# vismaychuriwala/Fast-Image-Editing-with-Generative-Models

Measured on AMD Instinct MI355X. Metric: PIE-Bench images/sec @1024^2 SSD-1B fp16 4-step, higher is better.
Workload: dtype f16; 1 GPU; ssd-1b fp16 + ControlNet-Canny(full) LCM img2img, num_inference_steps=4, strength=0.5, guidance=1.5, 1024x1024, batch=1 image per GPU, one edit at a time; unet_preset=ssd-1b-A1, controlnet_preset=controlnet-canny-sdxl-full, unet_evals=2, cfg_batch=2, parallelism=image-parallel x1, launch=hipGraph replay, weights=f16

## Files before the change

### fast-image-editing-with-generative-models_amd/csrc/gemm_common.h

```cpp
#pragma once
#include "fie_internal.h"
#include "gemm_addr.h"

namespace fie_gemm {

constexpr int BK = 64;

struct GemmArgs {
    const half_t* A1; int64_t lda1; int K1;
    const half_t* A2; int64_t lda2;
    const half_t* A3; int64_t lda3; int C2x, C3x; int64_t a3_bytes;
    int H, W, Cin, OH, OW, stride, pt, pl, ups;
    const half_t* Wt; int64_t ldw;
    half_t* C; int64_t ldc;
    int M, N, K;
    const half_t* bias;
    const half_t* rowbias; int64_t ld_rowbias; int rows_per_batch;
    const half_t* res; int64_t ldr;
    float scale; int act;
    int nbm, nbn;
    int64_t a1_bytes, a2_bytes, w_bytes;
    int taps2, oscat, opy, opx;
    int64_t w_par_stride;
    int gn_nch, gn_chunk0;
// ... 398 lines not shown
                    const float vq = lane == 0 ? tq[0] : lane == 1 ? tq[1] : lane == 2 ? tq[2] : tq[3];
                    float2* dst = reinterpret_cast<float2*>(p.gn_partial) + ((int64_t)b * nch + chunk) * p.gn_G + nfrag / p.gn_cg + lane;
                    *dst = make_float2(vs, vq);
                }
            }
        }
    }
    if constexpr (BUF) {
        if (p.out_f8) {
            const __amdgpu_buffer_rsrc_t rs8 = buf_rsrc(p.C, (int64_t)(p.M - 1) * p.ldc + (geglu ? p.N >> 1 : p.N));
            const float inv = p.out_inv_scale;
            auto q = [&](float x) { return fie_sat448(x * inv); };
#pragma unroll
            for (int j = 0; j < FM; ++j) {
                const int m = mrow + j * fld;
                const unsigned ro = m < p.M ? (unsigned)m * (unsigned)p.ldc : kRowOut;
#pragma unroll
                for (int i = 0; i < FN; ++i) {
                    const int n = ncol + i * 16;
                    if (geglu) {
                        const int pk = __builtin_amdgcn_cvt_pk_fp8_f32(q(acc[i][j][0]), q(acc[i][j][1]), 0, false);
                        __builtin_amdgcn_raw_buffer_store_b16((unsigned short)(pk & 0xffff), rs8, ro + (n < p.N ? (unsigned)(n >> 1) : kColOut), 0, 0);
                    } else {
                        int pk = __builtin_amdgcn_cvt_pk_fp8_f32(q(acc[i][j][0]), q(acc[i][j][1]), 0, false);
                        pk = __builtin_amdgcn_cvt_pk_fp8_f32(q(acc[i][j][2]), q(acc[i][j][3]), pk, true);
                        __builtin_amdgcn_raw_buffer_store_b32((unsigned)pk, rs8, ro + (n < p.N ? (unsigned)n : kColOut), 0, 0);
                    }
                }
            }
            return;
        }
    }
    const __amdgpu_buffer_rsrc_t rs_c = buf_rsrc(p.C, BUF ? ((int64_t)(p.oscat ? 4 * (int64_t)p.M : p.M) - 1) * p.ldc * 2 + (geglu ? p.N >> 1 : p.N) * 2 : 0);
#pragma unroll
    for (int j = 0; j < FM; ++j) {
        const int m = mrow + j * fld;
        const unsigned ro = coff_row(j);
#pragma unroll
        for (int i = 0; i < FN; ++i) {
            const int n = ncol + i * 16;
            if (geglu) {
                f16x2 o;
                o[0] = (half_t)acc[i][j][0]; o[1] = (half_t)acc[i][j][1];
                if constexpr (BUF) {
                    unsigned bits; __builtin_memcpy(&bits, &o, 4);
                    __builtin_amdgcn_raw_buffer_store_b32(bits, rs_c, ro + coff(i, true), 0, 0);
                } else if (m < p.M && n < p.N) {
                    *reinterpret_cast<f16x2*>(p.C + (int64_t)m * p.ldc + (n >> 1)) = o;
                }
            } else {
                f16x4 o;
#pragma unroll
                for (int r = 0; r < 4; ++r) o[r] = (half_t)acc[i][j][r];
                if constexpr (BUF) {
                    u32x2 bits; __builtin_memcpy(&bits, &o, 8);
                    __builtin_amdgcn_raw_buffer_store_b64(bits, rs_c, ro + coff(i, false), 0, 0);
                } else if (m < p.M && n < p.N) {
                    *reinterpret_cast<f16x4*>(p.C + (int64_t)m * p.ldc + n) = o;
                }
            }
        }
        __builtin_amdgcn_sched_barrier(0);
    }
}

constexpr unsigned kOob = 0x80000000u;

__device__ __forceinline__ void bload16(__amdgpu_buffer_rsrc_t rsrc, half_t* lds_dst, unsigned voff, unsigned soff) {
    __builtin_amdgcn_raw_ptr_buffer_load_lds(rsrc, (__attribute__((address_space(3))) void*)lds_dst, 16, voff, soff, 0, 0);
}

template <int N>
__device__ __forceinline__ void wait_vm() {
    static_assert(N >= 0 && N < 64, "vmcnt is a 6-bit counter");
    asm volatile("s_waitcnt vmcnt(%0)" ::"n"(N) : "memory");
}

template <int N>
__device__ __forceinline__ void wait_vm_barrier() {
    static_assert(N >= 0 && N < 64, "vmcnt is a 6-bit counter");
    asm volatile("s_waitcnt vmcnt(%0)\n\ts_barrier" ::"n"(N) : "memory");
}

template <int FM, int FN, int NW>
__device__ __forceinline__ bool splitk_reduce(const GemmArgs& p, f32x4 (&acc)[FN][FM], int tile, int slice, int tid, void* lds) {
    constexpr int kTile = FM * FN * NW * 64 * 4;
    const int S = p.splitk;
    float* base = p.sk_slabs + (size_t)tile * S * kTile;
    {
        const __amdgpu_buffer_rsrc_t rs = buf_rsrc(base + (size_t)slice * kTile, kTile * 4);
#pragma unroll
        for (int i = 0; i < FN; ++i)
#pragma unroll
            for (int j = 0; j < FM; ++j)
                __builtin_amdgcn_raw_buffer_store_b128(__builtin_bit_cast(u32x4, acc[i][j]), rs, (unsigned)((i * FM + j) * NW * 64 + tid) * 16u, 0, 16);
    }
    asm volatile("s_waitcnt vmcnt(0)" ::: "memory");
    __syncthreads();
    volatile unsigned* flag = reinterpret_cast<volatile unsigned*>(lds);
    if (tid == 0) *flag = __hip_atomic_fetch_add(p.sk_tickets + tile, 1u, __ATOMIC_RELAXED, __HIP_MEMORY_SCOPE_AGENT);
    __syncthreads();
    if (*flag % (unsigned)S != (unsigned)(S - 1)) return false;
    if (tid == 0) {
        (void)__hip_atomic_fetch_sub(p.sk_tickets + tile, (unsigned)S, __ATOMIC_RELAXED, __HIP_MEMORY_SCOPE_AGENT);
        __builtin_amdgcn_fence(__ATOMIC_ACQUIRE, "agent");
    }
    asm volatile("s_waitcnt vmcnt(0)" ::: "memory");
    __syncthreads();
#pragma unroll
    for (int i = 0; i < FN; ++i)
#pragma unroll
        for (int j = 0; j < FM; ++j) acc[i][j] = (f32x4){0.f, 0.f, 0.f, 0.f};
    for (int s = 0; s < S; ++s) {
        const __amdgpu_buffer_rsrc_t rs = buf_rsrc(base + (size_t)s * kTile, kTile * 4);
        u32x4 v[FN][FM];
#pragma unroll
        for (int i = 0; i < FN; ++i)
#pragma unroll
            for (int j = 0; j < FM; ++j) v[i][j] = __builtin_amdgcn_raw_buffer_load_b128(rs, (unsigned)((i * FM + j) * NW * 64 + tid) * 16u, 0, 16);
#pragma unroll
        for (int i = 0; i < FN; ++i)
#pragma unroll
            for (int j = 0; j < FM; ++j) acc[i][j] += __builtin_bit_cast(f32x4, v[i][j]);
    }
    return true;
}

__device__ __forceinline__ int xcd_remap(int bid, int nwg) {
    const int q = nwg >> 3, r = nwg & 7, xcd = bid & 7;
    return (xcd < r ? xcd * (q + 1) : r * (q + 1) + (xcd - r) * q) + (bid >> 3);
}

}

int fie_launch_gemm8(fie_ctx* ctx, const fie_gemm::GemmArgs& a, int conv, int split);
int fie_gemm8_init(void);
int fie_gemm_init(void);
int fie_launch_conv_halo(fie_ctx* ctx, fie_gemm::GemmArgs& a, int stamped);
bool fie_conv_halo_ok(const fie_gemm::GemmArgs& a);
bool fie_conv_halo_edge_ok(const fie_gemm::GemmArgs& a);
int64_t fie_conv_halo_patches(const fie_gemm::GemmArgs& a);
int fie_launch_conv_thin(fie_ctx* ctx, fie_gemm::GemmArgs& a);
bool fie_conv_thin_ok(const fie_gemm::GemmArgs& a);
bool fie_conv_halo_gna_ok(const fie_gemm::GemmArgs& a);
int fie_conv_halo_init(void);
int fie_launch_gemm_w8(fie_ctx* ctx, const fie_gemm::GemmArgs& a, int conv, int code);
int fie_gemm_w8_init(void);
int fie_launch_gemm_x8(fie_ctx* ctx, const fie_gemm::GemmArgs& a, int code, int conv);
int fie_gemm_x8_init(void);
```

### fast-image-editing-with-generative-models_amd/csrc/gemm_conv.hip

```cpp
#include <algorithm>
#include <cstdio>
#include <cstdlib>
#include <cstring>
#include <utility>

#include "gemm_common.h"
#include "gemm_tiles.h"

using namespace fie_gemm;

namespace {

template <int BM, int BN, int MODE>
__global__ __launch_bounds__(256) void gemm_kernel(GemmArgs p) {
    constexpr int WM = BM / 2, WN = BN / 2;
    constexpr int FM = WM / 16, FN = WN / 16;
    constexpr int RA = BM / 32, RW = BN / 32;
    __shared__ __attribute__((aligned(16))) half_t smem[2 * (BM + BN) * BK];

    const int tid = threadIdx.x;
    const int lane = tid & 63, wave = tid >> 6;
    const int wm = wave & 1, wn = wave >> 1;

    const int bid = xcd_remap(blockIdx.x, gridDim.x);
// ... 38 lines not shown
            }
            ci += BK;
            while (ci >= p.Cin) { ci -= p.Cin; ++tap; }
        } else {
            const bool k1 = k < p.K1;
            const half_t* src = k1 ? p.A1 : p.A2;
            const int64_t ld = k1 ? p.lda1 : p.lda2;
            const int kk = k1 ? k : k - p.K1;
#pragma unroll
            for (int i = 0; i < RA; ++i) {
                const bool ok = a_row[i].ok && k < p.K;
                ra[i] = ok ? *reinterpret_cast<const f16x8*>(src + a_base[i] * ld + kk) : zero8;
            }
        }
#pragma unroll
        for (int i = 0; i < RW; ++i)
            rw[i] = *reinterpret_cast<const f16x8*>(p.Wt + (int64_t)(n0 + r0 + 32 * i) * p.ldw + k);
    };
    auto store_tiles = [&](int buf) {
        half_t* sa = smem + buf * (BM + BN) * BK;
        half_t* sw = sa + BM * BK;
#pragma unroll
        for (int i = 0; i < RA; ++i) *reinterpret_cast<f16x8*>(sa + lds_off(r0 + 32 * i, c8)) = ra[i];
#pragma unroll
        for (int i = 0; i < RW; ++i) *reinterpret_cast<f16x8*>(sw + lds_off(r0 + 32 * i, c8)) = rw[i];
    };

    f32x4 acc[FN][FM];
#pragma unroll
    for (int i = 0; i < FN; ++i)
#pragma unroll
        for (int j = 0; j < FM; ++j) acc[i][j] = (f32x4){0.f, 0.f, 0.f, 0.f};

    const int nk = (p.K + BK - 1) / BK;
    load_tiles(0);
    store_tiles(0);
    __syncthreads();

    const int fr = lane & 15, fq = lane >> 4;
    for (int kt = 0; kt < nk; ++kt) {
        const int buf = kt & 1;
        if (kt + 1 < nk) load_tiles(kt + 1);
        const half_t* sa = smem + buf * (BM + BN) * BK;
        const half_t* sw = sa + BM * BK;
#pragma unroll
        for (int kk = 0; kk < 2; ++kk) {
            f16x8 fw[FN], fa[FM];
#pragma unroll
            for (int i = 0; i < FN; ++i)
                fw[i] = *reinterpret_cast<const f16x8*>(sw + lds_off(wn * WN + i * 16 + fr, kk * 4 + fq));
#pragma unroll
            for (int j = 0; j < FM; ++j)
                fa[j] = *reinterpret_cast<const f16x8*>(sa + lds_off(wm * WM + j * 16 + fr, kk * 4 + fq));
#pragma unroll
            for (int i = 0; i < FN; ++i)
#pragma unroll
                for (int j = 0; j < FM; ++j)
                    acc[i][j] = __builtin_amdgcn_mfma_f32_16x16x32_f16(fw[i], fa[j], acc[i][j], 0, 0, 0);
        }
        if (kt + 1 < nk) store_tiles(buf ^ 1);
        __syncthreads();
    }

    epilogue<FM, FN, WM, WN>(p, acc, m0, n0, wm, wn, lane);
}

template <int NP, int ST>
__device__ __forceinline__ void wait_stage(int later) {
    if (ST >= 3 && later >= 1) wait_vm_barrier<(ST >= 3 ? 1 : 0) * NP>();
    else wait_vm_barrier<0>();
}

template <int OFF>
__device__ __forceinline__ f16x8 lds_read16_async(unsigned addr) {
    f16x8 v;
    asm volatile("ds_read_b128 %0, %1 offset:%2" : "=v"(v) : "v"(addr), "n"(OFF));
    return v;
}
template <int N, int... I>
__device__ __forceinline__ void read_frags(f16x8 (&f)[N], unsigned addr, std::integer_sequence<int, I...>) {
    ((f[I] = lds_read16_async<I * 16 * BK * 2>(addr)), ...);
}

template <int BM, int BN, int ST, int MODE, int NW, bool PF = false, bool STAMP = false, bool ALT = false, int LEAN = 0>
__global__ __launch_bounds__(NW * 64) void gemm3_kernel(GemmArgs p) {
    constexpr bool LNF = LEAN == 2;
    static_assert(!LNF || (MODE == 0 && !STAMP), "LayerNorm fold: GEMM view only");
    static_assert(!ALT || (NW == 8 && MODE == 0 && !PF && !STAMP), "ALT: 8-wave GEMM-view tiles without the fragment prefetch");
    constexpr int WGN = (LEAN == 2 && BM * BN / (NW * 256) <= 16 && (BM / NW) % 16 == 0) ? 1 : (BN / (NW / 2)) % 16 == 0 ? NW / 2 : 1, WGM = NW / WGN;
    constexpr int WM = BM / WGM, WN = BN / WGN;
    constexpr int FM = WM / 16, FN = WN / 16;
    constexpr int NPW = BN / 8;
    constexpr int RA = BM / (8 * NW), RW = (NPW + NW - 1) / NW;
    constexpr int NP = RA + RW;
    constexpr int STAGE = (BM + BN) * BK;
    extern __shared__ __attribute__((aligned(16))) half_t smem[];

    const int tid = threadIdx.x;
    const int lane = tid & 63;
    const int wave = __builtin_amdgcn_readfirstlane(tid >> 6);
    const int wm = wave % WGM, wn = wave / WGM;

    const int bid_all = xcd_remap(blockIdx.x, gridDim.x);
    const int nsplit = p.splitk > 1 ? p.splitk : 1;
    const int tile_all = bid_all / nsplit, slice = bid_all - tile_all * nsplit;
    const int bid = take_parity(p, tile_all);
    const int m0 = (p.order ? bid % p.nbm : bid / p.nbn) * BM;
    const int n0 = (p.order ? bid / p.nbm : bid % p.nbn) * BN;
    const int lr = lane >> 3;
    const int c8 = (lane & 7) ^ lr;

    const int live = p.probe == 1 ? 0 : 1;
    const __amdgpu_buffer_rsrc_t rs_a1 = buf_rsrc(p.A1, (int)p.a1_bytes * live);
    const __amdgpu_buffer_rsrc_t rs_a2 = buf_rsrc(p.A2, (int)p.a2_bytes * live);
    const __amdgpu_buffer_rsrc_t rs_w = buf_rsrc(p.Wt, (int)p.w_bytes * live);
    const __amdgpu_buffer_rsrc_t rs_a3 = buf_rsrc(p.A3, (int)p.a3_bytes * live);
    const int lm0 = p.probe == 2 ? 0 : m0, ln0 = p.probe == 2 ? 0 : n0;

    unsigned a_off1[RA], a_off2[RA];
    unsigned a_off3[RA];
    const ConvGeom g = conv_geom(p, p.taps2);
    ConvRow a_row[RA];
    unsigned a_img[RA];
#pragma unroll
    for (int i = 0; i < RA; ++i) {
        const int m = lm0 + (wave + NW * i) * 8 + lr;
        if (MODE == 2) {
            a_row[i] = conv_row(g, m);
            a_img[i] = (unsigned)a_row[i].b * (unsigned)(p.H * p.W) * (unsigned)p.Cin * 2u;
            a_off1[i] = kOob;
            a_off2[i] = a_row[i].ok ? (unsigned)m * (unsigned)p.lda2 * 2u + c8 * 16u : kOob;
            a_off3[i] = a_row[i].ok ? (unsigned)m * (unsigned)p.lda3 * 2u + c8 * 16u : kOob;
        } else {
            a_off1[i] = a_off2[i] = a_off3[i] = a_img[i] = 0;
            a_row[i] = ConvRow{};
        }
    }
    const unsigned a_base1 = (unsigned)(lm0 + wave * 8 + lr) * (unsigned)p.lda1 * 2u + c8 * 16u;
    const unsigned a_base2 = (unsigned)(lm0 + wave * 8 + lr) * (unsigned)p.lda2 * 2u + c8 * 16u;
    const unsigned a_step1 = (unsigned)(NW * 8) * (unsigned)p.lda1 * 2u, a_step2 = (unsigned)(NW * 8) * (unsigned)p.lda2 * 2u;
    const unsigned w_base = (unsigned)(ln0 + wave * 8 + lr) * (unsigned)p.ldw * 2u + c8 * 16u;
    const unsigned w_step = (unsigned)(NW * 8) * (unsigned)p.ldw * 2u;

    const int csteps = MODE == 2 ? p.Cin / BK : 1;
    const int k1_steps = p.K1 / BK;
    const int nk_all = (p.K + BK - 1) / BK;
    const KSlice ks(nk_all, slice, nsplit, csteps);
    const int kbeg = ks.kbeg, nk = ks.nk;
    const bool ktail = (p.K % BK) != 0;
    int ftap = ks.ftap, cs = ks.cs;
    bool tap_fresh = true;

    const int ntaps = conv_taps(g);
    auto issue = [&](int kt, int stage) {
        half_t* sa = smem + stage * STAGE;
        if (MODE == 2 && ftap >= ntaps) {
            const int e = kt - ntaps * csteps, x2 = p.C2x / BK;
            if (e < x2) {
#pragma unroll
                for (int i = 0; i < RA; ++i) bload16(rs_a2, sa + (wave + NW * i) * 512, a_off2[i], (unsigned)e * (BK * 2));
            } else {
#pragma unroll
                for (int i = 0; i < RA; ++i) bload16(rs_a3, sa + (wave + NW * i) * 512, a_off3[i], (unsigned)(e - x2) * (BK * 2));
            }
        } else if (MODE == 2) {
            if (cs == 0 || tap_fresh) {
                tap_fresh = false;
                const TapYX t = tap_yx(g, ftap);
#pragma unroll
// ... 168 lines not shown
            fill = fill + 1 == ST ? 0 : fill + 1;
            asm volatile("s_waitcnt lgkmcnt(0)" ::: "memory");
            landed(fw1, fa1);
            if (kt + 1 < nk) {
                wait_stage<NP, ST>(min(kt + ST - 1, nk - 1) - (kt + 1));
                ln_pin();
                reads(fw0, fa0, stage, 0);
            }
            mfmas(fw1, fa1);
        }
    } else
    for (int kt = 0; kt < nk; ++kt) {
        const int later = min(kt + ST - 2, nk - 1) - kt;
        if constexpr (ALT && ST >= 3) {
            if (later >= 1 && kt >= ST - 1 && (kt & 1) != grp) wait_vm_barrier<2 * NP>();
            else wait_vm_barrier<0>();
        } else
        wait_stage<NP, ST>(later);
        stamp(kt == 0 ? 7 : 0);
        const bool more = kt + ST - 1 < nk;
        const half_t* sa = smem + stage * STAGE;
#pragma unroll
        for (int kk = 0; kk < 2; ++kk) {
            if (more && p.probe != 3) {
                if constexpr (ALT) {
                    if (kk == 0 && ((kt + ST - 1) & 1) == grp) issue_alt(kbeg + kt + ST - 1, fill);
                } else {
                    if (kk == 0) { issue(kbeg + kt + ST - 1, fill); if (NW != 8) issue_w(kbeg + kt + ST - 1, fill); }
                    else if (NW == 8) issue_w(kbeg + kt + ST - 1, fill);
                }
            }
            stamp(1 + 3 * kk);
            if constexpr (FM * FN > 16) {
                constexpr int HM = FM / 2;
                const half_t* sw = sa + BM * BK;
                f16x8 fw[FN];
#pragma unroll
                for (int i = 0; i < FN; ++i) fw[i] = *reinterpret_cast<const f16x8*>(sw + lds_off(wn * WN + i * 16 + fr, kk * 4 + fq));
#pragma unroll
                for (int jh = 0; jh < 2; ++jh) {
                    f16x8 fa[HM];
#pragma unroll
                    for (int j = 0; j < HM; ++j) fa[j] = *reinterpret_cast<const f16x8*>(sa + lds_off(wm * WM + (jh * HM + j) * 16 + fr, kk * 4 + fq));
                    __builtin_amdgcn_s_setprio(1);
                    static_for([&](auto ic) {
                        constexpr int i = decltype(ic)::value;
#pragma unroll
                        for (int j = 0; j < HM; ++j) acc[i][jh * HM + j] = __builtin_amdgcn_mfma_f32_16x16x32_f16(fw[i], fa[j], acc[i][jh * HM + j], 0, 0, 0);
                        if (jh == 0) ln_slice(ic, std::integral_constant<int, FN>{}, c0_t{}, std::integral_constant<int, HM>{}, fa);
                        else ln_slice(ic, std::integral_constant<int, FN>{}, std::integral_constant<int, HM>{}, std::integral_constant<int, HM>{}, fa);
                    }, std::make_integer_sequence<int, FN>{});
                    __builtin_amdgcn_s_setprio(0);
                }
            } else {
                f16x8 fw[FN], fa[FM];
                frags(fw, fa, sa, kk);
                if constexpr (STAMP) asm volatile("s_waitcnt lgkmcnt(0)" ::: "memory");
                stamp(2 + 3 * kk);
                mfmas(fw, fa);
                stamp(3 + 3 * kk);
            }
        }
        stage = stage + 1 == ST ? 0 : stage + 1;
        fill = fill + 1 == ST ? 0 : fill + 1;
    }
    stamp(11);
    float ln_mean[LNF ? FM : 1], ln_rstd[LNF ? FM : 1];
    if constexpr (LNF && FM * FN <= 16) {
#pragma unroll
        for (int i = 0; i < FN; ++i) ln_tab_load(p, n0 + wn * WN + i * 16 + (lane >> 4) * 4, ln_pre.lo[i], ln_pre.hi[i]);
    }
    if constexpr (LNF) {
        const float inv_k = 1.f / (float)p.K;
#pragma unroll
        for (int j = 0; j < FM; ++j) {
            float sx = ln_s[j], sq = ln_q[j];
            sx += __shfl_xor(sx, 16); sx += __shfl_xor(sx, 32);
            sq += __shfl_xor(sq, 16); sq += __shfl_xor(sq, 32);
            const float mu = sx * inv_k;
            ln_mean[j] = mu;
            ln_rstd[j] = rsqrtf(fmaxf(sq * inv_k - mu * mu, 0.f) + p.ln_eps);
        }
    }
    if constexpr (FM * FN <= 16 && !LEAN) {
        if (nsplit > 1 && !splitk_reduce<FM, FN, NW>(p, acc, tile_all, slice, tid, smem)) return;
    }
    if constexpr (LNF && FM * FN > 16) {
        epilogue_geglu_lean<FM, FN, WM, WN, true>(p, acc, m0, n0, wm, wn, lane, ln_mean, ln_rstd);
    } else if constexpr (LNF) {
        epilogue_lean_ln<FM, FN, WM, WN>(p, acc, m0, n0, wm, wn, lane, ln_pre, ln_mean, ln_rstd);
    } else
    if constexpr (FM * FN > 16) {
        if (p.act == FIE_ACT_GEGLU && p.epi_prefetch && !p.rowbias && !p.res && p.scale == 1.f && !p.gn_partial && !p.out_f8 && !p.w_scale && !p.oscat && p.probe == 0) {
            epilogue_geglu_lean<FM, FN, WM, WN>(p, acc, m0, n0, wm, wn, lane);
        } else {
        static_for([&](auto cc) {
            constexpr int C = decltype(cc)::value;
            epilogue<FM, 2, WM, WN, true>(p, reinterpret_cast<f32x4(&)[2][FM]>(acc[2 * C]), m0, n0 + 32 * C, wm, wn, lane);
        }, std::make_integer_sequence<int, FN / 2>{});
        if constexpr (FN & 1)
            epilogue<FM, 1, WM, WN, true>(p, reinterpret_cast<f32x4(&)[1][FM]>(acc[FN - 1]), m0, n0 + 16 * (FN - 1), wm, wn, lane);
        }
    } else {
        if constexpr (LEAN == 1) epilogue_lean<FM, FN, WM, WN>(p, acc, m0, n0, wm, wn, lane, pre);
        else epilogue<FM, FN, WM, WN, true>(p, acc, m0, n0, wm, wn, lane, &pre);
    }
    if constexpr (STAMP) {
        asm volatile("s_waitcnt vmcnt(0)" ::: "memory");
        stamp(8);
        seg[10] = tprev;
        if (p.stamps && lane == 0) {
#pragma unroll
            for (int i = 0; i < 12; ++i) p.stamps[((size_t)bid * NW + wave) * 12 + i] = seg[i];
        }
    }
}

enum Family { kGeneric, kRing, kPhased, kHalo, kHaloEdge, kThin };
enum : unsigned { kSplitK = 1, kStamps = 2, kGemmOnly = 4, kLnFold = 8, kPF = 16, kAlt = 32 };
using LaunchFn = int (*)(fie_ctx*, GemmArgs&, dim3 grid);
struct Tile {
    int code, bm, bn;
    Family family;
    const char* name;
    unsigned flags;
    int w8, x8;
    LaunchFn gemm, conv, ln;
    hipError_t (*attr)();
};

template <int BM, int BN, int ST, int NW, unsigned F = 0>
struct RingTile {
    static constexpr bool PF = F & kPF, STAMP = F & kStamps, ALT = F & kAlt;
    static constexpr int lds = ST * (BM + BN) * BK * (int)sizeof(half_t);
    template <int MODE>
    static constexpr bool has_lean = MODE == 0 && !STAMP && BM * BN / (NW * 64) <= 64;
    static_assert(!((F & kLnFold) && STAMP) && !((F & kSplitK) && (STAMP || BM * BN / (NW * 64) > 64)), "no LN fold or split-K with stamps; split-K on <= 16 fragments per lane");
    template <int MODE, int LEAN>
    static constexpr auto kernel() { return &gemm3_kernel<BM, BN, ST, MODE, NW, PF, STAMP, ALT, LEAN>; }
    template <int MODE, bool LN = false>
    static int launch(fie_ctx* ctx, GemmArgs& a, dim3 grid) {
        auto k = kernel<MODE, LN ? 2 : 0>();
        if constexpr (!LN && has_lean<MODE>) {
            if (a.epi_prefetch && a.splitk <= 1 && !a.rowbias && a.act == FIE_ACT_NONE && a.scale == 1.f && !a.gn_partial && !a.out_f8 && !a.w_scale && !a.oscat &&
                a.probe == 0)
                k = kernel<MODE, 1>();
        }
        fie_launch(ctx, k, grid, dim3(NW * 64), lds, a);
        FIE_LAUNCH_CHECK();
        return FIE_OK;
    }
    static hipError_t attr() {
        hipError_t e = hipSuccess;
        auto set = [&](auto* k) { if (e == hipSuccess) e = hipFuncSetAttribute(reinterpret_cast<const void*>(k), hipFuncAttributeMaxDynamicSharedMemorySize, lds); };
        set(kernel<0, 0>());
        if constexpr (has_lean<0>) set(kernel<0, 1>());
        if constexpr (!(F & kGemmOnly)) set(kernel<2, 0>());
        if constexpr (F & kLnFold) set(kernel<0, 2>());
        return e;
    }
    static constexpr Tile row(int code, const char* name, int w8, int x8) {
        Tile t = {code, BM, BN, kRing, name, F, w8, x8, &launch<0>, nullptr, nullptr, &attr};
        if constexpr (!(F & kGemmOnly)) t.conv = &launch<2>;
        if constexpr (F & kLnFold) t.ln = &launch<0, true>;
        return t;
    }
};

template <int BM, int BN, int MODE>
int launch_generic(fie_ctx* ctx, GemmArgs& a, dim3 grid) {
    fie_launch(ctx, (gemm_kernel<BM, BN, MODE>), grid, dim3(256), 0, a);
    FIE_LAUNCH_CHECK();
    return FIE_OK;
}
template <int BM, int BN>
constexpr Tile generic_row(int code, int w8, int x8) { return {code, BM, BN, kGeneric, "gemm_kernel", 0, w8, x8, &launch_generic<BM, BN, 0>, &launch_generic<BM, BN, 1>}; }
template <int CONV, int VARIANT>
int launch_phased(fie_ctx* ctx, GemmArgs& a, dim3) { return fie_launch_gemm8(ctx, a, CONV, VARIANT); }
template <int VARIANT>
int launch_halo(fie_ctx* ctx, GemmArgs& a, dim3) { return fie_launch_conv_halo(ctx, a, VARIANT); }
int launch_thin(fie_ctx* ctx, GemmArgs& a, dim3) { return fie_launch_conv_thin(ctx, a); }

constexpr Tile kTiles[] = {
    generic_row<128, 128>(1, 62, 43),
    generic_row<128, 64>(2, 42, 42),
    generic_row<64, 64>(3, 43, 43),
    RingTile<128, 64, 3, 4, kSplitK | kLnFold>::row(42, "gemm3_kernel", 42, 42),
    RingTile<64, 64, 3, 4, kSplitK>::row(43, "gemm3_kernel", 43, 43),
    RingTile<128, 64, 2, 4, kSplitK>::row(44, "gemm3_kernel", 42, 42),
    RingTile<64, 64, 2, 4, kSplitK>::row(46, "gemm3_kernel", 43, 43),
    RingTile<128, 96, 3, 4, kSplitK>::row(47, "gemm3_kernel", 62, 47),
    RingTile<128, 80, 3, 4, kSplitK>::row(48, "gemm3_kernel", 62, 0),
    RingTile<128, 128, 3, 8, kSplitK>::row(51, "gemm3_kernel", 62, 51),
    RingTile<128, 128, 2, 8, kSplitK>::row(52, "gemm3_kernel", 52, 52),
    RingTile<192, 128, 2, 8, kSplitK>::row(54, "gemm3_kernel", 54, 54),
    RingTile<256, 256, 2, 8>::row(61, "gemm3_kernel", 62, 62),
    RingTile<256, 128, 3, 8, kSplitK>::row(62, "gemm3_kernel", 62, 62),
    RingTile<256, 320, 2, 8, kGemmOnly>::row(63, "gemm3_kernel", 62, 63),
    RingTile<256, 320, 2, 8, kGemmOnly | kAlt | kLnFold>::row(64, "gemm3_kernel", 62, 63),
    RingTile<128, 128, 3, 8, kPF | kSplitK>::row(95, "gemm3_kernel+prefetch", 62, 51),
    RingTile<256, 128, 3, 8, kPF | kSplitK | kLnFold>::row(96, "gemm3_kernel+prefetch", 62, 62),
    RingTile<256, 128, 3, 8, kStamps>::row(97, "gemm3_kernel+prefetch", 62, 0),
    RingTile<256, 128, 3, 8, kPF | kStamps>::row(98, "gemm3_kernel+prefetch", 62, 0),
    RingTile<128, 64, 3, 4, kStamps>::row(94, "gemm3_kernel+prefetch", 62, 0),
    {81, 256, 256, kPhased, "gemm8_kernel", 0, 62, 62, &launch_phased<0, 0>, &launch_phased<1, 0>},
    {82, 256, 256, kPhased, "gemm8_kernel", 0, 62, 0, &launch_phased<0, 1>, &launch_phased<1, 1>},
    {71, 256, 128, kHalo, "conv_halo_kernel", 0, 62, 0, nullptr, &launch_halo<0>},
    {73, 256, 128, kHalo, "conv_halo_kernel", kStamps, 62, 0, nullptr, &launch_halo<1>},
    {72, 256, 128, kHalo, "conv_halo2_kernel", 0, 62, 0, nullptr, &launch_halo<2>},
    {74, 256, 128, kHalo, "conv_halo2_kernel", kStamps, 62, 0, nullptr, &launch_halo<4>},
    {76, 256, 128, kHalo, "conv_halo2_kernel", 0, 62, 0, nullptr, &launch_halo<5>},
    {78, 256, 128, kHaloEdge, "conv_halo2_kernel+edge", 0, 62, 0, nullptr, &launch_halo<6>},
    {77, 64, 16, kThin, "conv_thin_kernel", 0, 62, 0, &launch_thin, &launch_thin},
};
constexpr const Tile* find_tile(int code) {
    for (const Tile& t : kTiles)
        if (t.code == code) return &t;
    return nullptr;
}
constexpr bool is_family(int code, Family f) { return find_tile(code) && find_tile(code)->family == f; }

constexpr int kCandF16[] = {43, 46, 42, 44, 51, 52, 54, 96, 81, 63, 47, 48, 64, 72, 78};
constexpr int kCandW8[] = {43, 42, 62, 52, 54};
constexpr int kCandX8[] = {43, 42, 47, 51, 52, 54, 62, 63};
struct SplitCand { int code, per_cu; };
constexpr SplitCand kSplitF16[] = {{96, 1}, {95, 1}, {47, 1}, {54, 2}, {52, 2}};
constexpr SplitCand kSplitX8[] = {{62, 1}, {51, 1}, {47, 1}, {54, 2}, {52, 2}};

template <size_t N>
constexpr bool f8_built(const fie_f8_tile (&built)[N], int code) {
    const Tile* t = find_tile(code);
    for (const fie_f8_tile& b : built)
        if (t && b.code == code && b.bm == t->bm && b.bn == t->bn) return true;
    return false;
}
constexpr int table_error() {
    for (const Tile& t : kTiles) {
        int n = 0;
        for (const Tile& u : kTiles) n += u.code == t.code;
        if (n != 1) return 1;
        if (!f8_built(kFieW8Tiles, t.w8) || (t.x8 && !f8_built(kFieX8Tiles, t.x8))) return 2;
        if ((t.flags & kSplitK) && t.family != kRing) return 3;
        if ((!t.conv && !(t.flags & kGemmOnly)) || (!t.gemm && t.family != kHalo && t.family != kHaloEdge)) return 4;
    }
    for (int c : kCandF16) if (!find_tile(c)) return 5;
    for (int c : kCandW8) if (!f8_built(kFieW8Tiles, c)) return 6;
    for (int c : kCandX8) if (!f8_built(kFieX8Tiles, c)) return 7;
    for (const SplitCand& c : kSplitF16) if (!find_tile(c.code) || !(find_tile(c.code)->flags & kSplitK)) return 8;
    for (const SplitCand& c : kSplitX8) if (!f8_built(kFieX8Tiles, c.code) || !(find_tile(c.code)->flags & kSplitK)) return 9;
    return 0;
}
static_assert(table_error() == 0, "kTiles / candidate lists inconsistent: see table_error for the rule with that number");

template <int MODE>
int heuristic_code(const fie_ctx* ctx, const GemmArgs& a, bool dma_ok) {
    auto blocks = [&](int bm, int bn) { return (int64_t)((a.M + bm - 1) / bm) * ((a.N + bn - 1) / bn); };
    const int64_t cus = ctx->num_cus;
    const int64_t b256 = blocks(256, 256), b62 = blocks(256, 128), b51 = blocks(128, 128), b42 = blocks(128, 64);
    int code;
    if (!dma_ok) {
        code = b42 >= cus ? 2 : 3;
    } else if (MODE == 1 && fie_conv_halo_ok(a) && 4 * (int64_t)(a.M / 256) * ((a.N + 127) / 128) >= 3 * cus && a.C2x + a.C3x <= 4 * BK &&
               std::find(std::begin(ctx->tune_exclude), std::end(ctx->tune_exclude), 72) == std::end(ctx->tune_exclude)) {
        code = 72;
    } else if (MODE == 1 && fie_conv_halo_edge_ok(a) && 4 * fie_conv_halo_patches(a) * ((a.N + 127) / 128) >= 3 * cus && a.C2x + a.C3x <= 4 * BK &&
               std::find(std::begin(ctx->tune_exclude), std::end(ctx->tune_exclude), 78) == std::end(ctx->tune_exclude)) {
        code = 78;
    } else if (MODE == 1) {
        if (!a.A2 && ((b256 >= cus && (a.N % 256 == 0 || (a.N % 128 != 0 && a.K >= 5760))) ||
            (a.N % 256 == 0 && a.K >= 8192 && 2 * b256 >= cus))) code = 81;
        else if (a.N % 128 == 0 && b62 >= 150) code = 96;
        else if (a.N % 128 == 0 && a.K >= 5760 && b51 >= 100) code = 51;
        else if (2 * b42 < 3 * cus) code = 43;
        else code = 42;
    } else if (MODE == 0 && a.N % 320 == 0 && a.N >= 5120 && 4 * blocks(256, 320) >= 3 * cus) {
        code = 64;
    } else if (a.N % 256 == 0 && a.K >= 4096 && b256 >= cus) {
        code = 81;
    } else if (a.N % 128 == 0 && b62 >= 150 && (a.N >= 1536 || a.K >= 2048 || a.M >= 16384)) {
        code = 96;
    } else if (a.N >= 2048 && a.K >= 1024 && b51 >= cus) {
        code = 51;
    } else if (a.K <= 640 && a.N <= 640) {
        code = 43;
    } else if (b42 >= cus * 7 / 2 || a.K >= 4096 || (a.K >= 1024 && b42 >= cus)) {
        code = 42;
    } else {
        code = 43;
    }
    return code;
}

constexpr int64_t kSkTickets = 4096;

inline int splitk_fit(const fie_ctx* ctx, const GemmArgs& a, const Tile& t, int want) {
    const int bm = t.bm, bn = t.bn;
    if (want <= 1 || !(t.flags & kSplitK) || !ctx->sk_ws || !ctx->splitk_mode || (a.w_scale && a.a_scale == 0.f)) return 1;
    const int64_t tiles = (int64_t)((a.M + bm - 1) / bm) * ((a.N + bn - 1) / bn) * (a.oscat == 2 ? 4 : 1);
    const int nk = (a.K + BK - 1) / BK / (a.a_scale != 0.f ? 2 : 1);
    int s = want;
    while (s > 1 && (nk / s < 4 || tiles > kSkTickets || (int64_t)(kSkTickets * 4 + tiles * s * bm * bn * 4) > ctx->sk_bytes)) --s;
    return s;
}

template <int MODE>
int run_code(fie_ctx* ctx, GemmArgs& a, int code, int order, bool dma_ok, int split = 1) {
    const Tile* t = find_tile(code);
    FIE_REQUIRE(t != nullptr, "unknown tile code %d", code);
    const Family fam = t->family;
    FIE_REQUIRE(fam == kGeneric || fam == kThin || dma_ok, "tile code %d: shape not eligible for the LDS-DMA kernels (operands >= 2 GiB, Cin %% 64 != 0, or A = [A1 | A2] with K1 %% 64 != 0 or K %% 64 != 0)", code);
    FIE_REQUIRE(!(a.taps2 && (fam == kGeneric || a.w_scale)), "tile code %d: the 2x2 parity convs run on the f16 LDS-DMA kernels only", code);
    FIE_REQUIRE(!(MODE == 1 && a.A2 && (fam == kGeneric || fam == kPhased || a.w_scale)), "tile code %d: conv + 1x1 side inputs run on the f16 ring kernels and the halo-resident kernel (72) only", code);
    FIE_REQUIRE(!(fam == kHalo && (MODE != 1 || !dma_ok || !fie_conv_halo_ok(a))), "tile code %d (halo-resident conv): stride-1 same-size 3x3 conv with H, W %% 16 == 0, Cin %% 64 == 0, f16 weights only", code);
    FIE_REQUIRE(!(fam == kHaloEdge && (MODE != 1 || !dma_ok || !fie_conv_halo_edge_ok(a))), "tile code 78 (halo-resident conv, edge patches): stride-1 same-size 3x3 conv with H or W %% 16 != 0, "
                "Cin %% 64 == 0, Cin >= 128, N %% 64 == 0, f16 weights, no activation / scale / GroupNorm sums only");
    if (order < 0) {
        const int64_t nbm = (a.M + t->bm - 1) / t->bm, nbn = (a.N + t->bn - 1) / t->bn;
        const int64_t per_xcd = (nbm * nbn + 7) / 8;
        const double a_tile = (double)t->bm * a.K * 2 * (MODE == 1 ? 1.0 / 9 : 1.0), w_tile = (double)t->bn * a.K * 2;
        auto fabric = [&](int64_t fast, int64_t slow, double fast_tile, double slow_tile) {
            const int64_t rows = (per_xcd + fast - 1) / fast;
            return (double)(rows < slow ? rows : slow) * slow_tile + (double)(per_xcd < fast ? per_xcd : fast) * fast_tile;
        };
        order = fabric(nbm, nbn, a_tile, w_tile) < fabric(nbn, nbm, w_tile, a_tile) ? 1 : 0;
    }
    const bool x8 = a.w_scale && a.a_scale != 0.f;
    if (x8) {
        FIE_REQUIRE(dma_ok && !a.A2 && !a.taps2, "fp8 activations: plain GEMM / 3x3 conv views on the LDS-DMA kernels only");
        FIE_REQUIRE(t->x8 != 0, "tile code %d has no fp8-activation kernel", code);
        t = find_tile(t->x8);
        if (MODE == 1 && (t->flags & kGemmOnly)) t = find_tile(62);
    } else if (a.w_scale) {
        FIE_REQUIRE(dma_ok, "fp8 weights: shape not eligible for the LDS-DMA kernels (operands >= 2 GiB, Cin %% 64 != 0, or A = [A1 | A2] with K1 %% 64 != 0 or K %% 64 != 0)");
        t = find_tile(t->w8);
    }
    code = t->code;
    a.nbm = (a.M + t->bm - 1) / t->bm;
    a.nbn = (a.N + t->bn - 1) / t->bn;
    split = splitk_fit(ctx, a, *t, split);
    a.splitk = split;
    a.sk_tickets = static_cast<unsigned*>(ctx->sk_ws);
    a.sk_slabs = reinterpret_cast<float*>(static_cast<char*>(ctx->sk_ws) + kSkTickets * 4);
    a.order = order;
    a.probe = ctx->gemm_probe;
    a.epi_prefetch = ctx->epi_prefetch;
    a.stamps = (t->flags & kStamps) ? ctx->gemm_stamps : nullptr;
    if (x8) snprintf(ctx->last_kernel, sizeof(ctx->last_kernel), "gemm3x8_kernel<%dx%d> (gemm, fp8 activations x fp8 weights, tile code %d)", t->bm, t->bn, code);
    else if (a.w_scale) snprintf(ctx->last_kernel, sizeof(ctx->last_kernel), "gemm3w8_kernel<%dx%d> (%s, fp8 weights, tile code %d)", t->bm, t->bn, MODE == 1 ? "conv3x3" : "gemm", code);
    else snprintf(ctx->last_kernel, sizeof(ctx->last_kernel), "%s<%dx%d> (%s, tile code %d)", t->name, t->bm, t->bn, MODE == 1 ? "conv3x3" : "gemm", code);
    if (split > 1) snprintf(ctx->last_kernel + strlen(ctx->last_kernel) - 1, 24, ", split-K %d)", split);
    if (ctx->oplog) {
        char rebuild[256];
        snprintf(rebuild, sizeof(rebuild), " | b=%d pad=%d C2=%d C3=%d K1=%d parity=%d w8=%d bias=%d rowbias=%d rpb=%d res=%d act=%d scale=%.9g gn=%d gnrows=%d f8out=%d ln=%d gna=%d",
                 MODE == 1 ? a.M / (a.OH * a.OW) : 1, MODE == 1 && !a.taps2 && a.pt == 0 ? 1 : 0, a.C2x, a.C3x, a.K1, a.taps2, a.w_scale ? (a.a_scale != 0.f ? 2 : 1) : 0,
                 a.bias != nullptr, a.rowbias != nullptr, a.rowbias ? a.rows_per_batch : 0, a.res != nullptr, a.act, (double)a.scale, a.gn_partial ? a.gn_G : 0,
                 a.gn_partial ? a.gn_rows : 0, a.out_f8, a.ln_tab != nullptr, a.gna_tab != nullptr);
        if (MODE == 1)
            FIE_DESC(ctx, "conv M=%d N=%d K=%d in=%dx%dx%d s%d u%d%s%s code=%d flop=%.0f%s", a.M * (a.oscat == 2 ? 4 : 1), a.N, a.K, a.H, a.W, a.Cin, a.stride, a.ups,
                     a.taps2 ? " up2x-parity" : "", a.A2 ? " +1x1" : "", code + 10000 * (split > 1 ? split : 0), 2.0 * a.M * a.N * a.K * (a.oscat == 2 ? 4 : 1), rebuild);
        else
            FIE_DESC(ctx, "gemm M=%d N=%d K=%d act=%d%s%s%s code=%d flop=%.0f%s", a.M, a.N, a.K, a.act, a.res ? " +res" : "", a.ln_tab ? " +ln" : "", a.w_scale ? (a.a_scale != 0.f ? " a8w8" : " w8") : "",
                     code + 10000 * (split > 1 ? split : 0), 2.0 * a.M * a.N * a.K, rebuild);
    }
    if (x8) return fie_launch_gemm_x8(ctx, a, code, MODE == 1);
    if (a.w_scale) return fie_launch_gemm_w8(ctx, a, MODE == 1, code);
    const dim3 grid((unsigned)(a.nbm * a.nbn * (a.oscat == 2 ? 4 : 1) * split));
    if (a.ln_tab) {
        FIE_REQUIRE(MODE == 0 && t->ln && split == 1, "LayerNorm-folded GEMM: tile code %d not built for it", code);
        FIE_REQUIRE((code == 64) == (a.act == FIE_ACT_GEGLU), "LayerNorm-folded GEMM: GEGLU runs on tile 64 and nothing else does (code %d, act %d)", code, a.act);
        return t->ln(ctx, a, grid);
    }
    const LaunchFn fn = MODE == 1 ? t->conv : t->gemm;
    FIE_REQUIRE(fn != nullptr, "tile code %d (%dx%d%s) is built for the GEMM view only", code, t->bm, t->bn, (t->flags & kAlt) ? ", alternating refill" : "");
    return fn(ctx, a, grid);
}

constexpr size_t kFlushBytes = 384u << 20;

template <int MODE>
std::vector<int> tune_candidates(const fie_ctx* ctx, const GemmArgs& a, int guess) {
    static const bool use47 = !(getenv("FIE_TUNE_47") && getenv("FIE_TUNE_47")[0] == '0');
    std::vector<int> out;
    auto blocks = [&](int bm, int bn) { return (int64_t)((a.M + bm - 1) / bm) * ((a.N + bn - 1) / bn); };
// ... 624 lines not shown
```

Measured before the change: 14.92 images/sec.

## Specialize split-K kernels and fold peer slabs through a pipelined register ring

The split-K reducer no longer re-reads its own slab. It streams only the other slices' partial sums through a ring of in-flight buffer loads using packed f32 adds, and can pre-sum peer slabs before adding them to the accumulators. The split-K epilogue is moved into a separate SPLIT template instantiation, so non-split kernels drop that code and its register pressure, and the lean epilogue variant can now be combined with split-K. Split-K is capped at 4 ways to bound the specialisations, which may cut parallelism for shapes that previously used more slices.

```diff
diff --git a/fast-image-editing-with-generative-models_amd/csrc/gemm_common.h b/fast-image-editing-with-generative-models_amd/csrc/gemm_common.h
--- a/fast-image-editing-with-generative-models_amd/csrc/gemm_common.h
+++ b/fast-image-editing-with-generative-models_amd/csrc/gemm_common.h
@@ -504,11 +504,62 @@
     asm volatile("s_waitcnt vmcnt(%0)\n\ts_barrier" ::"n"(N) : "memory");
 }
 
+constexpr int kMaxSplitK = 4;
+
+typedef float f32x2 __attribute__((ext_vector_type(2)));
+__device__ __forceinline__ void sk_add(f32x4& a, const f32x4& b) {
+    f32x2 lo = __builtin_shufflevector(a, a, 0, 1), hi = __builtin_shufflevector(a, a, 2, 3);
+    asm volatile("v_pk_add_f32 %0, %0, %1" : "+v"(lo) : "v"(__builtin_shufflevector(b, b, 0, 1)));
+    asm volatile("v_pk_add_f32 %0, %0, %1" : "+v"(hi) : "v"(__builtin_shufflevector(b, b, 2, 3)));
+    a = __builtin_shufflevector(lo, hi, 0, 1, 2, 3);
+}
+__device__ __forceinline__ void sk_load_first(f32x4& slot, unsigned voff, u32x4 rs, unsigned soff) {
+    asm volatile("buffer_load_dwordx4 %0, %1, %2, %3 offen sc1" : "=v"(slot) : "v"(voff), "s"(rs), "s"(soff) : "memory");
+}
+__device__ __forceinline__ void sk_load_again(f32x4& slot, unsigned voff, u32x4 rs, unsigned soff) {
+    asm volatile("buffer_load_dwordx4 %0, %1, %2, %3 offen sc1" : "+v"(slot) : "v"(voff), "s"(rs), "s"(soff) : "memory");
+}
+
+template <int FM, int FN, int NW, int NF, int PRE>
+__device__ __forceinline__ void splitk_fold(f32x4 (&acc)[FN][FM], const float* base, int k, int tid) {
+    constexpr int kTile = FM * FN * NW * 64 * 4, NFR = FM * FN, NL = NFR * NF, RING = NFR < 8 ? NFR : 8;
+    static_assert(RING >= NF && NF >= 1 && NF <= 3 && PRE >= 1 && PRE <= NF, "a fragment's NF slots are all in the ring");
+    const uint64_t addr = reinterpret_cast<uint64_t>(base);
+    const u32x4 rs = {(unsigned)addr, (unsigned)(addr >> 32) & 0xffffu, (unsigned)((NF + 1) * kTile * 4), (unsigned)kBufRsrcFlags};
+    const unsigned voff = (unsigned)tid * 16u;
+    unsigned so[NF];
+#pragma unroll
+    for (int q = 0; q < NF; ++q) so[q] = (unsigned)(q + (q >= k ? 1 : 0)) * (unsigned)(kTile * 4);
+    f32x4 ring[RING];
+    auto soff = [&](int n) { return so[n % NF] + (unsigned)((n / NF) * NW * 1024); };
+    static_for([&](auto nc) {
+        constexpr int n = decltype(nc)::value;
+        sk_load_first(ring[n % RING], voff, rs, soff(n));
+    }, std::make_integer_sequence<int, (RING < NL ? RING : NL)>{});
+    static_for([&](auto fc) {
+        constexpr int f = decltype(fc)::value;
+        constexpr int issued = RING + f * NF < NL ? RING + f * NF : NL;
+        wait_vm<issued - (f + 1) * NF>();
+        f32x4& a = acc[f / FM][f % FM];
+        f32x4 &b0 = ring[(f * NF) % RING], &b1 = ring[(f * NF + (NF > 1 ? 1 : 0)) % RING], &b2 = ring[(f * NF + (NF > 2 ? 2 : 0)) % RING];
+        if constexpr (PRE >= 2) sk_add(b0, b1);
+        if constexpr (PRE >= 3) sk_add(b0, b2);
+        sk_add(a, b0);
+        if constexpr (NF > 1 && PRE < 2) sk_add(a, b1);
+        if constexpr (NF > 2 && PRE < 3) sk_add(a, b2);
+        static_for([&](auto qc) {
+            constexpr int n = f * NF + decltype(qc)::value + RING;
+            if constexpr (n < NL) sk_load_again(ring[n % RING], voff, rs, soff(n));
+        }, std::make_integer_sequence<int, NF>{});
+    }, std::make_integer_sequence<int, NFR>{});
+}
+
 template <int FM, int FN, int NW>
 __device__ __forceinline__ bool splitk_reduce(const GemmArgs& p, f32x4 (&acc)[FN][FM], int tile, int slice, int tid, void* lds) {
     constexpr int kTile = FM * FN * NW * 64 * 4;
     const int S = p.splitk;
     float* base = p.sk_slabs + (size_t)tile * S * kTile;
+    volatile unsigned* flag = reinterpret_cast<volatile unsigned*>(lds);
     {
         const __amdgpu_buffer_rsrc_t rs = buf_rsrc(base + (size_t)slice * kTile, kTile * 4);
 #pragma unroll
@@ -519,7 +570,6 @@
     }
     asm volatile("s_waitcnt vmcnt(0)" ::: "memory");
     __syncthreads();
-    volatile unsigned* flag = reinterpret_cast<volatile unsigned*>(lds);
     if (tid == 0) *flag = __hip_atomic_fetch_add(p.sk_tickets + tile, 1u, __ATOMIC_RELAXED, __HIP_MEMORY_SCOPE_AGENT);
     __syncthreads();
     if (*flag % (unsigned)S != (unsigned)(S - 1)) return false;
@@ -529,21 +579,15 @@
     }
     asm volatile("s_waitcnt vmcnt(0)" ::: "memory");
     __syncthreads();
-#pragma unroll
-    for (int i = 0; i < FN; ++i)
-#pragma unroll
-        for (int j = 0; j < FM; ++j) acc[i][j] = (f32x4){0.f, 0.f, 0.f, 0.f};
-    for (int s = 0; s < S; ++s) {
-        const __amdgpu_buffer_rsrc_t rs = buf_rsrc(base + (size_t)s * kTile, kTile * 4);
-        u32x4 v[FN][FM];
-#pragma unroll
-        for (int i = 0; i < FN; ++i)
-#pragma unroll
-            for (int j = 0; j < FM; ++j) v[i][j] = __builtin_amdgcn_raw_buffer_load_b128(rs, (unsigned)((i * FM + j) * NW * 64 + tid) * 16u, 0, 16);
-#pragma unroll
-        for (int i = 0; i < FN; ++i)
-#pragma unroll
-            for (int j = 0; j < FM; ++j) acc[i][j] += __builtin_bit_cast(f32x4, v[i][j]);
+    if (S == 2) splitk_fold<FM, FN, NW, 1, 1>(acc, base, slice, tid);
+    else if (S == 3) {
+        if (slice < 2) splitk_fold<FM, FN, NW, 2, 1>(acc, base, slice, tid);
+        else splitk_fold<FM, FN, NW, 2, 2>(acc, base, slice, tid);
+    } else {
+        static_assert(kMaxSplitK == 4, "one arm per (splitk, slices in front of the reducer's)");
+        if (slice < 2) splitk_fold<FM, FN, NW, 3, 1>(acc, base, slice, tid);
+        else if (slice == 2) splitk_fold<FM, FN, NW, 3, 2>(acc, base, slice, tid);
+        else splitk_fold<FM, FN, NW, 3, 3>(acc, base, slice, tid);
     }
     return true;
 }
diff --git a/fast-image-editing-with-generative-models_amd/csrc/gemm_conv.hip b/fast-image-editing-with-generative-models_amd/csrc/gemm_conv.hip
--- a/fast-image-editing-with-generative-models_amd/csrc/gemm_conv.hip
+++ b/fast-image-editing-with-generative-models_amd/csrc/gemm_conv.hip
@@ -144,9 +144,10 @@
     ((f[I] = lds_read16_async<I * 16 * BK * 2>(addr)), ...);
 }
 
-template <int BM, int BN, int ST, int MODE, int NW, bool PF = false, bool STAMP = false, bool ALT = false, int LEAN = 0>
+template <int BM, int BN, int ST, int MODE, int NW, bool PF = false, bool STAMP = false, bool ALT = false, int LEAN = 0, bool SPLIT = false>
 __global__ __launch_bounds__(NW * 64) void gemm3_kernel(GemmArgs p) {
     constexpr bool LNF = LEAN == 2;
+    static_assert(!SPLIT || (!LNF && !STAMP && BM * BN / (NW * 64) <= 64), "split-K: <= 16 accumulator fragments per lane, no LayerNorm fold, no stamps");
     static_assert(!LNF || (MODE == 0 && !STAMP), "LayerNorm fold: GEMM view only");
     static_assert(!ALT || (NW == 8 && MODE == 0 && !PF && !STAMP), "ALT: 8-wave GEMM-view tiles without the fragment prefetch");
     constexpr int WGN = (LEAN == 2 && BM * BN / (NW * 256) <= 16 && (BM / NW) % 16 == 0) ? 1 : (BN / (NW / 2)) % 16 == 0 ? NW / 2 : 1, WGM = NW / WGN;
@@ -481,7 +482,7 @@
             ln_rstd[j] = rsqrtf(fmaxf(sq * inv_k - mu * mu, 0.f) + p.ln_eps);
         }
     }
-    if constexpr (FM * FN <= 16 && !LEAN) {
+    if constexpr (SPLIT) {
         if (nsplit > 1 && !splitk_reduce<FM, FN, NW>(p, acc, tile_all, slice, tid, smem)) return;
     }
     if constexpr (LNF && FM * FN > 16) {
@@ -535,15 +536,23 @@
     template <int MODE>
     static constexpr bool has_lean = MODE == 0 && !STAMP && BM * BN / (NW * 64) <= 64;
     static_assert(!((F & kLnFold) && STAMP) && !((F & kSplitK) && (STAMP || BM * BN / (NW * 64) > 64)), "no LN fold or split-K with stamps; split-K on <= 16 fragments per lane");
-    template <int MODE, int LEAN>
-    static constexpr auto kernel() { return &gemm3_kernel<BM, BN, ST, MODE, NW, PF, STAMP, ALT, LEAN>; }
+    template <int MODE, int LEAN, bool SPLIT = false>
+    static constexpr auto kernel() { return &gemm3_kernel<BM, BN, ST, MODE, NW, PF, STAMP, ALT, LEAN, SPLIT>; }
     template <int MODE, bool LN = false>
     static int launch(fie_ctx* ctx, GemmArgs& a, dim3 grid) {
         auto k = kernel<MODE, LN ? 2 : 0>();
+        const bool lean = !LN && has_lean<MODE> && a.epi_prefetch && !a.rowbias && a.act == FIE_ACT_NONE && a.scale == 1.f && !a.gn_partial && !a.out_f8 && !a.w_scale &&
+                          !a.oscat && a.probe == 0;
         if constexpr (!LN && has_lean<MODE>) {
-            if (a.epi_prefetch && a.splitk <= 1 && !a.rowbias && a.act == FIE_ACT_NONE && a.scale == 1.f && !a.gn_partial && !a.out_f8 && !a.w_scale && !a.oscat &&
-                a.probe == 0)
-                k = kernel<MODE, 1>();
+            if (lean) k = kernel<MODE, 1>();
+        }
+        if constexpr (!LN && (F & kSplitK)) {
+            if (a.splitk > 1) {
+                k = kernel<MODE, 0, true>();
+                if constexpr (has_lean<MODE>) {
+                    if (lean) k = kernel<MODE, 1, true>();
+                }
+            }
         }
         fie_launch(ctx, k, grid, dim3(NW * 64), lds, a);
         FIE_LAUNCH_CHECK();
@@ -556,6 +565,11 @@
         if constexpr (has_lean<0>) set(kernel<0, 1>());
         if constexpr (!(F & kGemmOnly)) set(kernel<2, 0>());
         if constexpr (F & kLnFold) set(kernel<0, 2>());
+        if constexpr (F & kSplitK) {
+            set(kernel<0, 0, true>());
+            if constexpr (has_lean<0>) set(kernel<0, 1, true>());
+            if constexpr (!(F & kGemmOnly)) set(kernel<2, 0, true>());
+        }
         return e;
     }
     static constexpr Tile row(int code, const char* name, int w8, int x8) {
@@ -697,7 +711,7 @@
     if (want <= 1 || !(t.flags & kSplitK) || !ctx->sk_ws || !ctx->splitk_mode || (a.w_scale && a.a_scale == 0.f)) return 1;
     const int64_t tiles = (int64_t)((a.M + bm - 1) / bm) * ((a.N + bn - 1) / bn) * (a.oscat == 2 ? 4 : 1);
     const int nk = (a.K + BK - 1) / BK / (a.a_scale != 0.f ? 2 : 1);
-    int s = want;
+    int s = want < kMaxSplitK ? want : kMaxSplitK;
     while (s > 1 && (nk / s < 4 || tiles > kSkTickets || (int64_t)(kSkTickets * 4 + tiles * s * bm * bn * 4) > ctx->sk_bytes)) --s;
     return s;
 }
```

After: 15.00 images/sec, median of 6. Within noise of the previous version (+0.5%).
